# batra-mlp-lab/visdial

Hardware: NVIDIA H100
Metric: QA-rounds/sec mn-att-ques-im-hist+disc train step (higher is better)
Workload: dtype f16 operands + f16 saved state for the option LSTM, tf32 operands elsewhere; fp32 accumulate, fp32 cell state / gradients / optimiser

## Files before the change

visdial_b200/csrc/lstm16.cu:

```cuda
#include <cuda.h>
#include <cuda_fp16.h>
#include <map>
#include <mutex>
#include "../../include/visdial_b200.h"
#include "kernels.cuh"
#include "tc_ptx.cuh"

namespace vd {
namespace tc {

constexpr int BM16 = 128;
constexpr int BK16 = 64;
constexpr int UK16 = 16;
constexpr int BN16 = 128;
constexpr int EW16 = 8;
constexpr int STAGE16 = 32768;

__device__ __forceinline__ float tanh16(float x) { float y; asm("tanh.approx.f32 %0, %1;" : "=f"(y) : "f"(x)); return y; }
__device__ __forceinline__ float sig16(float x) { return fmaf(0.5f, tanh16(0.5f * x), 0.5f); }

__device__ __forceinline__ uint32_t pack2(float a, float b) {
  uint32_t r;
  asm("{\n .reg .f16 lo, hi;\n cvt.rn.satfinite.f16.f32 lo, %1;\n cvt.rn.satfinite.f16.f32 hi, %2;\n mov.b32 %0, {lo, hi};\n}"
      : "=r"(r) : "f"(a), "f"(b));
// ... 20 lines not shown
  unsigned lo = __shfl_sync(0xffffffffu, (unsigned)v, src_lane), hi = __shfl_sync(0xffffffffu, (unsigned)(v >> 32), src_lane);
  return (const void*)(((unsigned long long)hi << 32) | lo);
}
__device__ __forceinline__ void cp16(void* dst, const void* src) {
  asm volatile("cp.async.cg.shared.global [%0], [%1], 16;" ::"r"(smem_u32(dst)), "l"(src) : "memory");
}
__device__ __forceinline__ void t16_load(uint8_t* base, const void* mine, int lane) {
#pragma unroll
  for (int ps = 0; ps < 2; ++ps) {
    const int row = ps * 8 + (lane >> 2), c = lane & 3;
    const uint8_t* src = (const uint8_t*)shfl_vptr(mine, row);
    uint8_t* dst = base + row * 64 + ((c ^ ((row >> 1) & 3)) << 4);
    if (src) cp16(dst, src + c * 16); else *reinterpret_cast<uint4*>(dst) = make_uint4(0, 0, 0, 0);
  }
}
__device__ __forceinline__ void t32_load(uint8_t* base, const void* mine, int lane) {
#pragma unroll
  for (int ps = 0; ps < 4; ++ps) {
    const int row = ps * 4 + (lane >> 3), c = lane & 7;
    const uint8_t* src = (const uint8_t*)shfl_vptr(mine, row);
    uint8_t* dst = base + row * 128 + ((c ^ (row & 7)) << 4);
    if (src) cp16(dst, src + c * 16); else *reinterpret_cast<float4*>(dst) = make_float4(0.f, 0.f, 0.f, 0.f);
  }
}
__device__ __forceinline__ void cp_wait_all() {
  asm volatile("cp.async.wait_all;" ::: "memory");
  __syncwarp();
}
__device__ __forceinline__ float2 ld_h2(uint8_t* p) { return __half22float2(*reinterpret_cast<const __half2*>(p)); }
__device__ __forceinline__ void st_h2(uint8_t* p, float a, float b) { *reinterpret_cast<uint32_t*>(p) = pack2(a, b); }

struct Lstm16Params {
  int R, H;
  const __half* ptable; const int32_t* tok;
  const float* bias;
  const float* c_prev;
  const int32_t* mask_ids;
  float* h32_out;
  int save_gates;
  const __half* gsave; const float* c_cur; float* dc_carry;
};
struct Lstm16Maps { CUtensorMap g16, c, h16; };

template <int MODE>
struct Cfg16 {
  static constexpr int THREADS = 128 + 32 * EW16;
  static constexpr int STG_PER_WARP = MODE == 0 ? (5 * T16_BYTES + T32_BYTES) : (4 * T16_BYTES + 3 * T32_BYTES);
  static constexpr int STG_BYTES = EW16 * STG_PER_WARP;
  static constexpr int STAGES = (232448 - 1024 - 256 - STG_BYTES) / STAGE16;
  static constexpr int TOTAL = STAGES * STAGE16 + STG_BYTES + 1024 + 256;
};

template <int MODE>
__global__ void __launch_bounds__(Cfg16<MODE>::THREADS, 1)
k_lstm16(const __grid_constant__ CUtensorMap tmA, const __grid_constant__ CUtensorMap tmB,
         const __grid_constant__ Lstm16Maps em, const Lstm16Params p) {
  using C = Cfg16<MODE>;
  constexpr int STAGES = C::STAGES;
  extern __shared__ uint8_t smem_raw[];
  uint8_t* smem = (uint8_t*)(((uintptr_t)smem_raw + 1023) & ~(uintptr_t)1023);
  uint8_t* stg_all = smem + STAGES * STAGE16;
  uint64_t* full = (uint64_t*)(stg_all + C::STG_BYTES);
  uint64_t* empty = full + STAGES;

  const int warp = threadIdx.x >> 5, lane = threadIdx.x & 31;
  const int H = p.H;
  const int num_m = (p.R + BM16 - 1) / BM16;
  const int num_n = MODE == 0 ? H / 32 : H / BN16;
  const int num_tiles = num_m * num_n;
  const int num_kb = (MODE == 0 ? H : 4 * H) / BK16;

  if (threadIdx.x == 0) {
    for (int s = 0; s < STAGES; ++s) { mbar_init(&full[s], 1); mbar_init(&empty[s], 2); }
    asm volatile("fence.mbarrier_init.release.cluster;" ::: "memory");
  }
  __syncthreads();

  if (warp < 4) {
    if (threadIdx.x == 0) {
      int s = 0; uint32_t ph = 0;
      for (int tile = blockIdx.x; tile < num_tiles; tile += gridDim.x) {
        const int m0 = (tile / num_n) * BM16;
        const int nt = tile % num_n;
        for (int kb = 0; kb < num_kb; ++kb) {
          mbar_wait(&empty[s], ph ^ 1);
          uint8_t* sa = smem + s * STAGE16;
          uint8_t* sb = sa + 16384;
          mbar_expect_tx(&full[s], STAGE16);
          tma_load_2d(sa, &tmA, &full[s], kb * BK16, m0);
          if (MODE == 0) {
#pragma unroll
            for (int g = 0; g < 4; ++g) tma_load_2d(sb + g * 4096, &tmB, &full[s], kb * BK16, g * H + nt * 32);
          } else {
            tma_load_2d(sb, &tmB, &full[s], kb * BK16, nt * BN16);
          }
          if (++s == STAGES) { s = 0; ph ^= 1; }
        }
      }
    }
  } else {
    const int cw = warp - 4, wg = cw >> 2;
    uint8_t* stg = stg_all + cw * C::STG_PER_WARP;
    const int fr = lane >> 2, fu = 2 * (lane & 3);
    int s = 0; uint32_t ph = 0;
    auto contract = [&](float (&d)[BN16 / 2]) {
#pragma unroll
      for (int i = 0; i < BN16 / 2; ++i) d[i] = 0.f;
      int prev = -1;
      for (int kb = 0; kb < num_kb; ++kb) {
        mbar_wait(&full[s], ph);
        const uint32_t sa = smem_u32(smem + s * STAGE16);
        const uint64_t adesc = make_desc(sa + wg * 64 * 128, 16, 1024), bdesc = make_desc(sa + 16384, 16, 1024);
        wgmma_fence();
#pragma unroll
        for (int k = 0; k < BK16 / UK16; ++k)
          wgmma_f16_n128(d, adesc + (uint64_t)(k * 2), bdesc + (uint64_t)(k * 2), (kb | k) ? 1u : 0u);
        wgmma_commit();
        wgmma_wait<1>();
        if (prev >= 0 && (threadIdx.x & 127) == 0) mbar_arrive(&empty[prev]);
        prev = s;
        if (++s == STAGES) { s = 0; ph ^= 1; }
      }
      wgmma_wait<0>();
      wgmma_hold(d);
      if (prev >= 0 && (threadIdx.x & 127) == 0) mbar_arrive(&empty[prev]);
    };
    if constexpr (MODE == 0) {
      uint8_t* sG = stg; uint8_t* sH = stg + 4 * T16_BYTES; uint8_t* sC = sH + T16_BYTES;
      for (int tile = blockIdx.x; tile < num_tiles; tile += gridDim.x) {
        const int m0 = (tile / num_n) * BM16;
        const int nt = tile % num_n;
        const int r0 = m0 + wg * 64 + (cw & 3) * 16;
        const int j0 = nt * 32;
        const int64_t row = (int64_t)r0 + (lane & 15);
        const bool row_ok = row < p.R;
        const float keep = (row_ok && p.mask_ids && p.mask_ids[row] == 0) ? 0.f : 1.f;
        const int32_t tk = row_ok ? __ldg(p.tok + row) : 0;
        const __half* prow = tk != 0 ? p.ptable + (int64_t)tk * 4 * H + j0 : nullptr;
        const float* cprow = (row_ok && p.c_prev) ? p.c_prev + row * H + j0 : nullptr;
        if (lane == 0) bulk_wait_read0();
        __syncwarp();
#pragma unroll
        for (int g = 0; g < 4; ++g) t16_load(sG + g * T16_BYTES, prow ? prow + g * H : nullptr, lane);
        t32_load(sC, cprow, lane);
        float d[BN16 / 2];
        contract(d);
        cp_wait_all();
#pragma unroll
        for (int hh = 0; hh < 2; ++hh) {
          const int r = fr + 8 * hh;
          const float kp = __shfl_sync(0xffffffffu, keep, r);
          const int64_t grow = (int64_t)r0 + r;
#pragma unroll
          for (int jj = 0; jj < 4; ++jj) {
            const int u = 8 * jj + fu;
            float a[4][2], cp[2], hn[2];
#pragma unroll
            for (int g = 0; g < 4; ++g) {
              const float2 x = ld_h2(t16_at(sG + g * T16_BYTES, r, u));
              const float2 b = __ldg(reinterpret_cast<const float2*>(p.bias + g * H + j0 + u));
              a[g][0] = d[4 * (jj + 4 * g) + 2 * hh] + (x.x + b.x);
              a[g][1] = d[4 * (jj + 4 * g) + 2 * hh + 1] + (x.y + b.y);
            }
            const float2 c2 = *reinterpret_cast<const float2*>(t32_at(sC, r, u));
            cp[0] = c2.x; cp[1] = c2.y;
#pragma unroll
            for (int e = 0; e < 2; ++e) {
              const float gi = sig16(a[0][e]), gf = sig16(a[1][e]), go = sig16(a[2][e]), gg = tanh16(a[3][e]);
              const float c_ = (gf * cp[e] + gi * gg) * kp;
              a[0][e] = gi * kp; a[1][e] = gf * kp; a[2][e] = go * kp; a[3][e] = gg * kp;
              cp[e] = c_; hn[e] = go * tanh16(c_) * kp;
            }
#pragma unroll
            for (int g = 0; g < 4; ++g) st_h2(t16_at(sG + g * T16_BYTES, r, u), a[g][0], a[g][1]);
            *reinterpret_cast<float2*>(t32_at(sC, r, u)) = make_float2(cp[0], cp[1]);
            st_h2(t16_at(sH, r, u), hn[0], hn[1]);
            if (p.h32_out && grow < p.R)
              *reinterpret_cast<float2*>(p.h32_out + grow * H + j0 + u) = make_float2(hn[0], hn[1]);
          }
        }
        fence_proxy_async_smem();
        __syncwarp();
        if (lane == 0) {
          if (p.save_gates) {
#pragma unroll
            for (int g = 0; g < 4; ++g) tma_store_2d(&em.g16, sG + g * T16_BYTES, g * H + j0, r0);
          }
          tma_store_2d(&em.c, sC, j0, r0);
          tma_store_2d(&em.h16, sH, j0, r0);
          bulk_commit();
        }
        __syncwarp();
      }
    } else {
      uint8_t* sG = stg; uint8_t* sCP = stg + 4 * T16_BYTES; uint8_t* sCC = sCP + T32_BYTES; uint8_t* sDC = sCC + T32_BYTES;
      for (int tile = blockIdx.x; tile < num_tiles; tile += gridDim.x) {
        const int m0 = (tile / num_n) * BM16;
        const int nt = tile % num_n;
        const int r0 = m0 + wg * 64 + (cw & 3) * 16;
        const int64_t row = (int64_t)r0 + (lane & 15);
        const bool row_ok = row < p.R;
        const float keep = (row_ok && p.mask_ids && p.mask_ids[row] == 0) ? 0.f : 1.f;
        const __half* grow = row_ok ? p.gsave + row * 4 * H : nullptr;
        const float* cprow = (row_ok && p.c_prev) ? p.c_prev + row * H : nullptr;
        const float* ccrow = row_ok ? p.c_cur + row * H : nullptr;
        const float* dcrow = row_ok ? p.dc_carry + row * H : nullptr;
        auto fetch = [&](int j) {
          if (lane == 0) bulk_wait_read0();
          __syncwarp();
#pragma unroll
          for (int g = 0; g < 4; ++g) t16_load(sG + g * T16_BYTES, grow ? grow + g * H + j : nullptr, lane);
          t32_load(sCP, cprow ? cprow + j : nullptr, lane);
          t32_load(sCC, ccrow ? ccrow + j : nullptr, lane);
          t32_load(sDC, dcrow ? dcrow + j : nullptr, lane);
        };
        fetch(nt * BN16);
        float d[BN16 / 2];
        contract(d);
#pragma unroll
        for (int grp = 0; grp < BN16 / 32; ++grp) {
          const int j = nt * BN16 + grp * 32;
          if (grp > 0) fetch(j);
          cp_wait_all();
#pragma unroll
          for (int hh = 0; hh < 2; ++hh) {
            const int r = fr + 8 * hh;
            const float keep_r = __shfl_sync(0xffffffffu, keep, r);
#pragma unroll
            for (int jj = 0; jj < 4; ++jj) {
              const int u = 8 * jj + fu;
              float g[4][2], cp[2], cc[2], dc[2], out[4][2], dcn[2];
#pragma unroll
              for (int gg = 0; gg < 4; ++gg) {
                const float2 x = ld_h2(t16_at(sG + gg * T16_BYTES, r, u));
                g[gg][0] = x.x; g[gg][1] = x.y;
              }
              const float2 cp2 = *reinterpret_cast<const float2*>(t32_at(sCP, r, u));
              const float2 cc2 = *reinterpret_cast<const float2*>(t32_at(sCC, r, u));
              const float2 dc2 = *reinterpret_cast<const float2*>(t32_at(sDC, r, u));
              cp[0] = cp2.x; cp[1] = cp2.y; cc[0] = cc2.x; cc[1] = cc2.y; dc[0] = dc2.x; dc[1] = dc2.y;
#pragma unroll
              for (int e = 0; e < 2; ++e) {
                const float dh = d[4 * (4 * grp + jj) + 2 * hh + e];
                const float gi = g[0][e], gf = g[1][e], go = g[2][e], gg_ = g[3][e];
                const float tcv = tanh16(cc[e]);
                const float dd = (dc[e] + dh * go * (1.f - tcv * tcv)) * keep_r;
                const float dhe = dh * keep_r;
                out[0][e] = dd * gg_ * gi * (1.f - gi);
                out[1][e] = dd * cp[e] * gf * (1.f - gf);
                out[2][e] = dhe * tcv * go * (1.f - go);
                out[3][e] = dd * gi * (1.f - gg_ * gg_);
                dcn[e] = dd * gf;
              }
#pragma unroll
              for (int gg = 0; gg < 4; ++gg) st_h2(t16_at(sG + gg * T16_BYTES, r, u), out[gg][0], out[gg][1]);
              *reinterpret_cast<float2*>(t32_at(sDC, r, u)) = make_float2(dcn[0], dcn[1]);
            }
          }
          fence_proxy_async_smem();
          __syncwarp();
          if (lane == 0) {
#pragma unroll
            for (int gg = 0; gg < 4; ++gg) tma_store_2d(&em.g16, sG + gg * T16_BYTES, gg * H + j, r0);
            tma_store_2d(&em.c, sDC, j, r0);
            bulk_commit();
          }
          __syncwarp();
        }
      }
    }
    if (lane == 0) asm volatile("cp.async.bulk.wait_group 0;" ::: "memory");
  }
}

constexpr int A16_KB = 64;
constexpr int A16_BM = 128, A16_BN = 256;
constexpr int A16_THREADS = 384;
constexpr int A16_A_BYTES = (A16_BM / 64) * A16_KB * 128;
constexpr int A16_B_BYTES = (A16_BN / 64) * A16_KB * 128;
constexpr int A16_STAGE = A16_A_BYTES + A16_B_BYTES;
constexpr int A16_STAGES = 4;
constexpr int A16_TOTAL = A16_STAGES * A16_STAGE + 1024 + 256;
constexpr int A16_CHUNKS_PER_CTA = 24;
constexpr int A16_MIN_CHUNK = 32;
struct Atb16Params {
  int M, N, tiles_n, tiles, kbt;
  int chunk, num_chunks;
  float* C; int64_t ldc; const float* inv_scale;
  int* counter;
};

// ... 258 lines not shown
#pragma unroll
      for (int e = 0; e < 8; ++e) acc[e] += v[e];
    }
    flush(cur);
  }
}

static CUtensorMap make_tmap16(const void* base, CUtensorMapDataType dt, int esize, int64_t rows, int64_t cols, int64_t ld,
                               int box_rows, int box_cols, CUtensorMapSwizzle swz) {
  CUtensorMap tm;
  cuuint64_t dims[2] = {(cuuint64_t)cols, (cuuint64_t)rows};
  cuuint64_t strides[1] = {(cuuint64_t)ld * esize};
  cuuint32_t box[2] = {(cuuint32_t)box_cols, (cuuint32_t)box_rows};
  cuuint32_t estr[2] = {1, 1};
  CUresult r = get_encode()(&tm, dt, 2, (void*)base, dims, strides, box, estr, CU_TENSOR_MAP_INTERLEAVE_NONE, swz,
                            CU_TENSOR_MAP_L2_PROMOTION_L2_256B, CU_TENSOR_MAP_FLOAT_OOB_FILL_NONE);
  if (r != CUDA_SUCCESS) {
    char buf[256];
    snprintf(buf, sizeof(buf), "cuTensorMapEncodeTiled (lstm16) failed (%d): base %p rows %lld cols %lld ld %lld box %dx%d", (int)r, base,
             (long long)rows, (long long)cols, (long long)ld, box_rows, box_cols);
    throw CudaError(-3, buf);
  }
  return tm;
}
static CUtensorMap tmap_h(const __half* base, int64_t rows, int64_t cols, int64_t ld, int box_rows, int box_cols,
                          CUtensorMapSwizzle swz) {
  return make_tmap16(base, CU_TENSOR_MAP_DATA_TYPE_FLOAT16, 2, rows, cols, ld, box_rows, box_cols, swz);
}
static CUtensorMap tmap_f(const float* base, int64_t rows, int64_t cols, int64_t ld, int box_rows, int box_cols,
                          CUtensorMapSwizzle swz) {
  return make_tmap16(base, CU_TENSOR_MAP_DATA_TYPE_FLOAT32, 4, rows, cols, ld, box_rows, box_cols, swz);
}

template <int MODE>
static void launch16(LaunchCtx& cx, const CUtensorMap& tA, const CUtensorMap& tB, const Lstm16Maps& em, const Lstm16Params& p,
                     int num_tiles) {
  using C = Cfg16<MODE>;
  static bool attr_set = false;
  if (!attr_set) {
    VD_CUDA_CHECK(cudaFuncSetAttribute(k_lstm16<MODE>, cudaFuncAttributeMaxDynamicSharedMemorySize, C::TOTAL));
    attr_set = true;
  }
  const int pmax = cx.sms();
  int grid = num_tiles;
  if (num_tiles > pmax) { const int rounds = cdiv(num_tiles, pmax); grid = cdiv(num_tiles, rounds); }
  k_lstm16<MODE><<<grid, C::THREADS, C::TOTAL, cx.stream>>>(tA, tB, em, p);
  check_launch(cx, "k_lstm16");
}

}

bool lstm16_shape_ok(int64_t R, int H) { return H % 256 == 0 && H <= 512 && R >= 1024; }

void lstm16_step_fwd(LaunchCtx& cx, int64_t R, int H, const __half* h_prev16, const __half* Wh16, const __half* ptable16,
                     const int32_t* tok, const float* bias, const float* c_prev, const int32_t* mask_ids, __half* gates16,
                     float* c_out, __half* h16_out, float* h32_out) {
  using namespace tc;
  VD_REQUIRE(lstm16_shape_ok(R, H), VD_E_STATE, "lstm16_step_fwd: shape");
  Lstm16Params p = {};
  p.R = (int)R; p.H = H; p.ptable = ptable16; p.tok = tok; p.bias = bias; p.c_prev = c_prev; p.mask_ids = mask_ids;
  p.h32_out = h32_out; p.save_gates = gates16 != nullptr;
  CUtensorMap tA = tmap_h(h_prev16, R, H, H, BM16, BK16, CU_TENSOR_MAP_SWIZZLE_128B);
  CUtensorMap tB = tmap_h(Wh16, 4 * (int64_t)H, H, H, 32, BK16, CU_TENSOR_MAP_SWIZZLE_128B);
  Lstm16Maps em;
  em.g16 = gates16 ? tmap_h(gates16, R, 4 * (int64_t)H, 4 * (int64_t)H, 16, 32, CU_TENSOR_MAP_SWIZZLE_64B)
                   : tmap_h(h16_out, R, H, H, 16, 32, CU_TENSOR_MAP_SWIZZLE_64B);
  em.c = tmap_f(c_out, R, H, H, 16, 32, CU_TENSOR_MAP_SWIZZLE_128B);
  em.h16 = tmap_h(h16_out, R, H, H, 16, 32, CU_TENSOR_MAP_SWIZZLE_64B);
  launch16<0>(cx, tA, tB, em, p, cdiv(R, BM16) * (H / 32));
}

void lstm16_step_bwd(LaunchCtx& cx, int64_t R, int H, const __half* da_next16, const __half* Whb16, const __half* gates16,
                     const float* c_prev, const float* c_cur, float* dc_carry, const int32_t* mask_ids, __half* da16) {
  using namespace tc;
  VD_REQUIRE(lstm16_shape_ok(R, H), VD_E_STATE, "lstm16_step_bwd: shape");
  Lstm16Params p = {};
  p.R = (int)R; p.H = H; p.gsave = gates16; p.c_prev = c_prev; p.c_cur = c_cur; p.dc_carry = dc_carry; p.mask_ids = mask_ids;
  CUtensorMap tA = tmap_h(da_next16, R, 4 * (int64_t)H, 4 * (int64_t)H, BM16, BK16, CU_TENSOR_MAP_SWIZZLE_128B);
// ... 18 lines not shown
  const int64_t n = R * (H / 8);
  tc::k_lstm16_bwd_last<<<(unsigned)((n + 255) / 256), 256, 0, cx.stream>>>(gates16, c_prev, c_cur, dh_last, scale, mask_ids,
                                                                             dc_carry, da16, R, H);
  check_launch(cx, "k_lstm16_bwd_last");
}

void cvt_f32_to_f16(LaunchCtx& cx, __half* dst, int64_t ldd, const float* src, int64_t lds, int64_t rows, int cols) {
  VD_REQUIRE(cols % 4 == 0 && lds % 4 == 0 && ldd % 4 == 0, VD_E_STATE, "cvt_f32_to_f16: alignment");
  const int64_t n = rows * (cols / 4);
  if (n == 0) return;
  tc::k_cvt16<<<(unsigned)((n + 255) / 256), 256, 0, cx.stream>>>(dst, ldd, src, lds, rows, cols);
  check_launch(cx, "k_cvt16");
}

void pick_grad_scale(LaunchCtx& cx, const float* x, int64_t n, uint32_t* bits, float* scale2) {
  VD_REQUIRE(n % 4 == 0, VD_E_STATE, "pick_grad_scale: n % 4");
  VD_CUDA_CHECK(cudaMemsetAsync(bits, 0, sizeof(uint32_t), cx.stream));
  const int blocks = (int)std::min<int64_t>((n / 4 + 255) / 256, 4 * cx.sm_count);
  tc::k_amax<<<blocks, 256, 0, cx.stream>>>(x, n / 4, bits);
  check_launch(cx, "k_amax");
  tc::k_pick_scale<<<1, 1, 0, cx.stream>>>(bits, scale2);
  check_launch(cx, "k_pick_scale");
}

void segsum_rows16(LaunchCtx& cx, const __half* X, int64_t ldx, const int32_t* perm, const int32_t* sorted_tok, int64_t n,
                   float* out, int ncols, const float* inv_scale) {
  VD_REQUIRE(ncols % 8 == 0 && ldx % 8 == 0, VD_E_STATE, "segsum_rows16: alignment");
  if (n == 0) return;
  tc::k_segsum16<<<(unsigned)((n + tc::SEG16_ROWS - 1) / tc::SEG16_ROWS), 256, 0, cx.stream>>>(X, ldx, perm, sorted_tok, n, out, ncols,
                                                                                               inv_scale);
  check_launch(cx, "k_segsum16");
}

static int* atb16_counter(cudaStream_t stream) {
  static std::mutex mu;
  static std::map<std::pair<int, cudaStream_t>, int*> counters;
  int dev = 0;
  VD_CUDA_CHECK(cudaGetDevice(&dev));
  std::lock_guard<std::mutex> lock(mu);
  int*& c = counters[{dev, stream}];
  if (!c) {
    VD_CUDA_CHECK(cudaMalloc((void**)&c, 2 * sizeof(int)));
    VD_CUDA_CHECK(cudaMemsetAsync(c, 0, 2 * sizeof(int), stream));
  }
  return c;
}

void gemm_atb16(LaunchCtx& cx, int M, int N, int64_t K, const __half* A, int64_t lda, const __half* B, int64_t ldb, float* C,
                int64_t ldc, const float* inv_scale) {
  using namespace tc;
  VD_REQUIRE(M % 64 == 0 && N % 64 == 0 && K >= A16_KB && lda % 8 == 0 && ldb % 8 == 0, VD_E_STATE, "gemm_atb16: shape");
  Atb16Params p = {};
  p.M = M; p.N = N; p.tiles_n = cdiv(N, A16_BN); p.tiles = cdiv(M, A16_BM) * p.tiles_n;
  VD_REQUIRE((K + A16_KB - 1) / A16_KB <= INT32_MAX, VD_E_STATE, "gemm_atb16: K");
  p.kbt = (int)((K + A16_KB - 1) / A16_KB);
  const int64_t sms = cx.sms(), total = (int64_t)p.tiles * p.kbt;
  p.chunk = (int)std::min<int64_t>(p.kbt, std::max<int64_t>(A16_MIN_CHUNK, cdiv(total, sms * A16_CHUNKS_PER_CTA)));
  p.num_chunks = p.tiles * cdiv(p.kbt, p.chunk);
  p.C = C; p.ldc = ldc; p.inv_scale = inv_scale;
  p.counter = atb16_counter(cx.stream);
  CUtensorMap tA = tmap_h(A, K, M, lda, A16_KB, 64, CU_TENSOR_MAP_SWIZZLE_128B),
              tB = tmap_h(B, K, N, ldb, A16_KB, 64, CU_TENSOR_MAP_SWIZZLE_128B);
  static bool attr_set = false;
  if (!attr_set) {
    VD_CUDA_CHECK(cudaFuncSetAttribute(k_atb16<true>, cudaFuncAttributeMaxDynamicSharedMemorySize, A16_TOTAL));
    VD_CUDA_CHECK(cudaFuncSetAttribute(k_atb16<false>, cudaFuncAttributeMaxDynamicSharedMemorySize, A16_TOTAL));
    attr_set = true;
  }
  const unsigned grid = (unsigned)std::min<int64_t>(sms, p.num_chunks);
  if (ldc % 4 == 0 && ((uintptr_t)C & 15) == 0) k_atb16<true><<<grid, A16_THREADS, A16_TOTAL, cx.stream>>>(tA, tB, p);
  else k_atb16<false><<<grid, A16_THREADS, A16_TOTAL, cx.stream>>>(tA, tB, p);
  check_launch(cx, "k_atb16");
}

}
```

visdial_b200/csrc/tc_ptx.cuh:

```cuda
#pragma once
#include <cuda.h>
#include <stdint.h>

namespace vd {
namespace tc {

__device__ __forceinline__ uint32_t smem_u32(const void* p) { return (uint32_t)__cvta_generic_to_shared(p); }

__device__ __forceinline__ void mbar_init(uint64_t* bar, uint32_t count) {
  asm volatile("mbarrier.init.shared::cta.b64 [%0], %1;" ::"r"(smem_u32(bar)), "r"(count));
}
__device__ __forceinline__ void mbar_expect_tx(uint64_t* bar, uint32_t bytes) {
  asm volatile("mbarrier.arrive.expect_tx.shared::cta.b64 _, [%0], %1;" ::"r"(smem_u32(bar)), "r"(bytes) : "memory");
}
__device__ __forceinline__ void mbar_arrive(uint64_t* bar) {
  asm volatile("mbarrier.arrive.shared::cta.b64 _, [%0];" ::"r"(smem_u32(bar)) : "memory");
}
__device__ __forceinline__ void mbar_wait(uint64_t* bar, uint32_t parity) {
  uint32_t done = 0, spins = 0;
  uint32_t addr = smem_u32(bar);
  while (!done) {
    asm volatile(
        "{\n .reg .pred p;\n mbarrier.try_wait.parity.shared::cta.b64 p, [%1], %2;\n selp.u32 %0, 1, 0, p;\n}"
        : "=r"(done) : "r"(addr), "r"(parity) : "memory");
    if (!done && ++spins > (1u << 24)) __trap();
  }
}
__device__ __forceinline__ void tma_load_2d(void* smem_dst, const CUtensorMap* tm, uint64_t* bar, int c0, int c1) {
  asm volatile(
      "cp.async.bulk.tensor.2d.shared::cluster.global.mbarrier::complete_tx::bytes [%0], [%1, {%3, %4}], [%2];"
      ::"r"(smem_u32(smem_dst)), "l"(tm), "r"(smem_u32(bar)), "r"(c0), "r"(c1) : "memory");
}
__device__ __forceinline__ void wgmma_fence() { asm volatile("wgmma.fence.sync.aligned;" ::: "memory"); }
__device__ __forceinline__ void wgmma_commit() { asm volatile("wgmma.commit_group.sync.aligned;" ::: "memory"); }
template <int N> __device__ __forceinline__ void wgmma_wait() { asm volatile("wgmma.wait_group.sync.aligned %0;" ::"n"(N) : "memory"); }
template <int NR> __device__ __forceinline__ void wgmma_hold(float (&d)[NR]) {
#pragma unroll
  for (int i = 0; i < NR; ++i) asm volatile("" : "+f"(d[i])::"memory");
}
__device__ __forceinline__ void bar_named(int id, int threads) { asm volatile("bar.sync %0, %1;" ::"r"(id), "r"(threads) : "memory"); }

__device__ __forceinline__ uint64_t make_desc(uint32_t saddr, uint32_t lbo_bytes, uint32_t sbo_bytes) {
  uint64_t d = 0;
  d |= (uint64_t)((saddr & 0x3FFFF) >> 4);
  d |= (uint64_t)((lbo_bytes >> 4) & 0x3FFF) << 16;
  d |= (uint64_t)((sbo_bytes >> 4) & 0x3FFF) << 32;
  d |= (uint64_t)1 << 62;
  return d;
}

__device__ __forceinline__ void wgmma_tf32_n32(float (&d)[16], uint64_t a, uint64_t b, uint32_t acc) {
  asm volatile(
      "{\n .reg .pred p;\n setp.ne.b32 p, %18, 0;\n"
      "wgmma.mma_async.sync.aligned.m64n32k8.f32.tf32.tf32 {%0, %1, %2, %3, %4, %5, %6, %7, %8, %9, %10, %11, %12, %13, %14, %15}, %16, %17, p, 1, 1;\n}\n"
      : "+f"(d[0]), "+f"(d[1]), "+f"(d[2]), "+f"(d[3]), "+f"(d[4]), "+f"(d[5]), "+f"(d[6]), "+f"(d[7]), "+f"(d[8]), "+f"(d[9]), "+f"(d[10]), "+f"(d[11]), "+f"(d[12]), "+f"(d[13]), "+f"(d[14]), "+f"(d[15])
      : "l"(a), "l"(b), "r"(acc));
}

__device__ __forceinline__ void wgmma_tf32_n64(float (&d)[32], uint64_t a, uint64_t b, uint32_t acc) {
  asm volatile(
      "{\n .reg .pred p;\n setp.ne.b32 p, %34, 0;\n"
      "wgmma.mma_async.sync.aligned.m64n64k8.f32.tf32.tf32 {%0, %1, %2, %3, %4, %5, %6, %7, %8, %9, %10, %11, %12, %13, %14, %15, %16, %17, %18, %19, %20, %21, %22, %23, %24, %25, %26, %27, %28, %29, %30, %31}, %32, %33, p, 1, 1;\n}\n"
      : "+f"(d[0]), "+f"(d[1]), "+f"(d[2]), "+f"(d[3]), "+f"(d[4]), "+f"(d[5]), "+f"(d[6]), "+f"(d[7]), "+f"(d[8]), "+f"(d[9]), "+f"(d[10]), "+f"(d[11]), "+f"(d[12]), "+f"(d[13]), "+f"(d[14]), "+f"(d[15]), "+f"(d[16]), "+f"(d[17]), "+f"(d[18]), "+f"(d[19]), "+f"(d[20]), "+f"(d[21]), "+f"(d[22]), "+f"(d[23]), "+f"(d[24]), "+f"(d[25]), "+f"(d[26]), "+f"(d[27]), "+f"(d[28]), "+f"(d[29]), "+f"(d[30]), "+f"(d[31])
      : "l"(a), "l"(b), "r"(acc));
}

__device__ __forceinline__ void wgmma_tf32_n128(float (&d)[64], uint64_t a, uint64_t b, uint32_t acc) {
  asm volatile(
      "{\n .reg .pred p;\n setp.ne.b32 p, %66, 0;\n"
      "wgmma.mma_async.sync.aligned.m64n128k8.f32.tf32.tf32 {%0, %1, %2, %3, %4, %5, %6, %7, %8, %9, %10, %11, %12, %13, %14, %15, %16, %17, %18, %19, %20, %21, %22, %23, %24, %25, %26, %27, %28, %29, %30, %31, %32, %33, %34, %35, %36, %37, %38, %39, %40, %41, %42, %43, %44, %45, %46, %47, %48, %49, %50, %51, %52, %53, %54, %55, %56, %57, %58, %59, %60, %61, %62, %63}, %64, %65, p, 1, 1;\n}\n"
      : "+f"(d[0]), "+f"(d[1]), "+f"(d[2]), "+f"(d[3]), "+f"(d[4]), "+f"(d[5]), "+f"(d[6]), "+f"(d[7]), "+f"(d[8]), "+f"(d[9]), "+f"(d[10]), "+f"(d[11]), "+f"(d[12]), "+f"(d[13]), "+f"(d[14]), "+f"(d[15]), "+f"(d[16]), "+f"(d[17]), "+f"(d[18]), "+f"(d[19]), "+f"(d[20]), "+f"(d[21]), "+f"(d[22]), "+f"(d[23]), "+f"(d[24]), "+f"(d[25]), "+f"(d[26]), "+f"(d[27]), "+f"(d[28]), "+f"(d[29]), "+f"(d[30]), "+f"(d[31]), "+f"(d[32]), "+f"(d[33]), "+f"(d[34]), "+f"(d[35]), "+f"(d[36]), "+f"(d[37]), "+f"(d[38]), "+f"(d[39]), "+f"(d[40]), "+f"(d[41]), "+f"(d[42]), "+f"(d[43]), "+f"(d[44]), "+f"(d[45]), "+f"(d[46]), "+f"(d[47]), "+f"(d[48]), "+f"(d[49]), "+f"(d[50]), "+f"(d[51]), "+f"(d[52]), "+f"(d[53]), "+f"(d[54]), "+f"(d[55]), "+f"(d[56]), "+f"(d[57]), "+f"(d[58]), "+f"(d[59]), "+f"(d[60]), "+f"(d[61]), "+f"(d[62]), "+f"(d[63])
      : "l"(a), "l"(b), "r"(acc));
// ... 72 lines not shown
```

visdial_b200/csrc/engine.h:

```cpp
#pragma once
#include <functional>
#include <string>
#include <vector>
#include "../../include/visdial_b200.h"
#include "kernels.cuh"

namespace vd {

enum EncKind { ENC_LF_QUES = 0, ENC_LF_QIH = 1, ENC_HREA = 2, ENC_MN_ATT = 3, ENC_LF_QI = 4, ENC_LF_QH = 5, ENC_HRE_QH = 6, ENC_HRE_QIH = 7,
               ENC_MN_QH = 8, ENC_MN_QIH = 9, ENC_LF_ATT = 10 };
enum DecKind { DEC_DISC = 0, DEC_GEN = 1 };

struct Cfg {
  std::string encoder, decoder;
  int enc = 0, dec = 0;
  int V = 0, E = 300, H = 512, L = 2, F = 4096, S = 14, IE = 300, Cm = 512, hops = 1, R = 10, K = 100;
  float dropout = 0.5f;
  int gpuid = 0;
  bool useIm = false, useHist = false, att = false;
  bool fam_lf = false, fam_hre = false, fam_mn = false;
  bool hre_att = false;
  bool san = false;
  bool img_in_q = false;
  bool img_drop = false;
// ... 153 lines not shown
  DropCfg dropcfg(float p) const;
  void gemm_tn(int M, int N, int K, const float* A, int64_t lda, const int32_t* gather, const float* B, int64_t ldb,
               float* C, int64_t ldc, float beta, const float* bias, int act);
  void gemm_atb(int M, int N, int64_t K, const float* A, int64_t lda, const int32_t* gather, const float* B, int64_t ldb,
                float* C, int64_t ldc);
  void linear_fwd(int wseg, const float* x, int64_t rows, float* y, int act);
  void linear_bwd(int wseg, const float* x, const float* dy, int64_t rows, float* dx, float beta_dx);
  void refresh_shadows();
  void stage_batch(const vd_batch* b);
  LstmRoute route_lstm(int64_t R, int H, bool gathered, bool has_h0, const float* WhT, int64_t ldw, const float* Wh) const;
  LstmRoute route_lstm(const LstmRun& r) const {
    return route_lstm(r.R, r.H, r.gather != nullptr, r.h0 != nullptr, Wtp(r.wseg) + r.D, r.D + r.H,
                      Wp(r.wseg) + (int64_t)r.D * 4 * r.H);
  }
  void route_lstm_pair(LstmRun& l1, LstmRun& l2) const;
  void lstm_simt_fwd_step(const LstmFwdStep& s);
  int lstm_tc_fwd_step(const LstmFwdStep& s);
  void lstm_simt_bwd_step(const LstmBwdStep& s);
  int lstm_tc_bwd_step(const LstmBwdStep& s);
  void lstm_forward(LstmRun& r, bool save);
  void lstm_forward_begin(LstmRun& r, bool save, bool xproj_by_caller = false);
  void lstm_forward_step(LstmRun& r, int t, bool xproj_by_caller = false);
  void lstm_xproj(const LstmRun& r, int t0, int nt, float* gates);
  void lstm_backward_begin(LstmRun& r, const float* dh_all, const float* dh_last, const float* dc_last);
  void lstm_backward_step(LstmRun& r, int t);
  void lstm_backward_end(LstmRun& r, float* dx_out, float* dh0_out, float* dc0_out);
  void lstm_pair_forward(LstmRun& l1, LstmRun& l2, const PairStreams& s);
  void lstm_pair_backward(LstmRun& l1, LstmRun& l2, const float* dh_last2, const float* dc_last2, const float* dh_last1,
                          const float* dc_last1, float* dx1_out, const PairStreams& s);
  bool serial_pairs() const { return cfg.useHist && hist1.route.fwd == LstmPath::Pair16; }
  cudaStream_t opt_stream = nullptr;
  cudaEvent_t ev_opt_fork = nullptr, ev_opt_done = nullptr;
  bool opt_overlap = true, opt_fwd_pending = false, opt_bwd_pending = false;
  int opt_reserve_sms = 16;
  float* opt_demb = nullptr;
  void options_forward_async();
  void options_backward(const float* dfeat);
  void join_options_backward();
  const int32_t* dense_round = nullptr;
  GrowBuf dense_buf[2];
  float forward_backward_dense(const vd_batch* b, const int32_t* round_host, const float* relevance_host);
  std::vector<cudaEvent_t> ev_pool;
  cudaEvent_t pool_event(size_t i);
  void lstm_backward(LstmRun& r, const float* dh_all, const float* dh_last, const float* dc_last, float* dx_out,
                     float* dh0_out, float* dc0_out);

  void encoder_forward(const vd_batch* b);
  void encoder_backward(const float* dEnc);
  float *qi_join = nullptr, *qi_proj = nullptr;
  const float* mn_query_in = nullptr;
  void mn_block_fwd(const float* qin, const float* h3, float* out);
  void mn_block_bwd(const float* dout, const float* out, float* dqin, float* dh3);
  void san_block_fwd(const float* u0);
  void san_block_bwd(const float* dEnc, float* du0);
  void forward_connect();
  void decoder_forward();
  float criterion_forward();
  void criterion_backward();
  void decoder_backward();
  const float* backward_connect();
  void retrieve(const vd_batch* b, int use_gt, int32_t* ranks_host);
  void gen_option_lhood();
  LstmRun gstep1, gstep2;
  float* gstep_logp = nullptr;
  void gen_decoder_step(int64_t rows, const int32_t* tokens_host, const float* const* h_prev, const float* const* c_prev);
  void gen_decoder_step_logits(int64_t rows, const int32_t* tok, const float* const* h_prev, const float* const* c_prev);
  void gen_beam_search(int k, int L, int start_token, int end_token, int32_t* answer_host, int32_t* length_host, double* score_host);
// ... 43 lines not shown
```

Baseline: 16150.

## Split option-LSTM kernel into dedicated MMA and epilogue warpgroups with smem accumulator handoff

Adds a separate MMA warpgroup that computes both 64-row halves of the 128x128 tile and hands the fp32 accumulators to eight epilogue warps through a shared-memory buffer guarded by full/empty mbarriers. The aim is to overlap the gate nonlinearity and backward epilogue of one tile with the tensor-core contraction of the next. Registers are rebalanced with setmaxnreg, and in backward mode c_prev is read directly into registers instead of being staged. The accumulator buffer takes shared memory, which can reduce the number of pipeline stages, and the single accumulator buffer still serialises MMA against epilogue reads.

```diff
diff --git a/visdial_b200/csrc/lstm16.cu b/visdial_b200/csrc/lstm16.cu
--- a/visdial_b200/csrc/lstm16.cu
+++ b/visdial_b200/csrc/lstm16.cu
@@ -88,12 +88,44 @@
 
 template <int MODE>
 struct Cfg16 {
-  static constexpr int THREADS = 128 + 32 * EW16;
-  static constexpr int STG_PER_WARP = MODE == 0 ? (5 * T16_BYTES + T32_BYTES) : (4 * T16_BYTES + 3 * T32_BYTES);
+  static constexpr int THREADS = 256 + 32 * EW16;
+  static constexpr int STG_PER_WARP = MODE == 0 ? (5 * T16_BYTES + T32_BYTES) : (4 * T16_BYTES + 2 * T32_BYTES);
   static constexpr int STG_BYTES = EW16 * STG_PER_WARP;
-  static constexpr int STAGES = (232448 - 1024 - 256 - STG_BYTES) / STAGE16;
-  static constexpr int TOTAL = STAGES * STAGE16 + STG_BYTES + 1024 + 256;
+  static constexpr int ACC_BYTES = BM16 * BN16 * 4;
+  static constexpr int STAGES = (232448 - 1024 - 256 - STG_BYTES - ACC_BYTES) / STAGE16;
+  static constexpr int TOTAL = STAGES * STAGE16 + ACC_BYTES + STG_BYTES + 1024 + 256;
 };
+
+template <int STAGES>
+__device__ __forceinline__ void contract16(float (&d)[2][BN16 / 2], uint8_t* smem, uint64_t* full, uint64_t* empty, int& s,
+                                           uint32_t& ph, int num_kb) {
+#pragma unroll
+  for (int j = 0; j < 2; ++j)
+#pragma unroll
+    for (int i = 0; i < BN16 / 2; ++i) d[j][i] = 0.f;
+  int prev = -1;
+  for (int kb = 0; kb < num_kb; ++kb) {
+    mbar_wait(&full[s], ph);
+    const uint32_t sa = smem_u32(smem + s * STAGE16);
+    const uint64_t bdesc = make_desc(sa + 16384, 16, 1024);
+    wgmma_fence();
+#pragma unroll
+    for (int k = 0; k < BK16 / UK16; ++k)
+#pragma unroll
+      for (int j = 0; j < 2; ++j)
+        wgmma_f16_n128(d[j], make_desc(sa + j * 64 * 128, 16, 1024) + (uint64_t)(k * 2), bdesc + (uint64_t)(k * 2),
+                       (kb | k) ? 1u : 0u);
+    wgmma_commit();
+    wgmma_wait<1>();
+    if (prev >= 0 && (threadIdx.x & 127) == 0) mbar_arrive(&empty[prev]);
+    prev = s;
+    if (++s == STAGES) { s = 0; ph ^= 1; }
+  }
+  wgmma_wait<0>();
+#pragma unroll
+  for (int j = 0; j < 2; ++j) wgmma_hold(d[j]);
+  if (prev >= 0 && (threadIdx.x & 127) == 0) mbar_arrive(&empty[prev]);
+}
 
 template <int MODE>
 __global__ void __launch_bounds__(Cfg16<MODE>::THREADS, 1)
@@ -103,9 +135,12 @@
   constexpr int STAGES = C::STAGES;
   extern __shared__ uint8_t smem_raw[];
   uint8_t* smem = (uint8_t*)(((uintptr_t)smem_raw + 1023) & ~(uintptr_t)1023);
-  uint8_t* stg_all = smem + STAGES * STAGE16;
+  float2* accbuf = (float2*)(smem + STAGES * STAGE16);
+  uint8_t* stg_all = smem + STAGES * STAGE16 + C::ACC_BYTES;
   uint64_t* full = (uint64_t*)(stg_all + C::STG_BYTES);
   uint64_t* empty = full + STAGES;
+  uint64_t* acc_full = empty + STAGES;
+  uint64_t* acc_empty = acc_full + 1;
 
   const int warp = threadIdx.x >> 5, lane = threadIdx.x & 31;
   const int H = p.H;
@@ -115,12 +150,15 @@
   const int num_kb = (MODE == 0 ? H : 4 * H) / BK16;
 
   if (threadIdx.x == 0) {
-    for (int s = 0; s < STAGES; ++s) { mbar_init(&full[s], 1); mbar_init(&empty[s], 2); }
+    for (int s = 0; s < STAGES; ++s) { mbar_init(&full[s], 1); mbar_init(&empty[s], 1); }
+    mbar_init(acc_full, 128);
+    mbar_init(acc_empty, 32 * EW16);
     asm volatile("fence.mbarrier_init.release.cluster;" ::: "memory");
   }
   __syncthreads();
 
   if (warp < 4) {
+    setmaxnreg_dec<40>();
     if (threadIdx.x == 0) {
       int s = 0; uint32_t ph = 0;
       for (int tile = blockIdx.x; tile < num_tiles; tile += gridDim.x) {
@@ -142,33 +180,28 @@
         }
       }
     }
+  } else if (warp < 8) {
+    setmaxnreg_inc<168>();
+    float2* mine = accbuf + ((warp - 4) * (BN16 / 4)) * 32 + lane;
+    int s = 0; uint32_t ph = 0, aph = 0;
+    for (int tile = blockIdx.x; tile < num_tiles; tile += gridDim.x) {
+      float d[2][BN16 / 2];
+      contract16<STAGES>(d, smem, full, empty, s, ph, num_kb);
+      mbar_wait(acc_empty, aph ^ 1);
+#pragma unroll
+      for (int e = 0; e < 2; ++e)
+#pragma unroll
+        for (int q = 0; q < BN16 / 4; ++q) mine[(e * 4 * (BN16 / 4) + q) * 32] = make_float2(d[e][2 * q], d[e][2 * q + 1]);
+      mbar_arrive(acc_full);
+      aph ^= 1;
+    }
   } else {
-    const int cw = warp - 4, wg = cw >> 2;
+    setmaxnreg_inc<152>();
+    const int cw = warp - 8, wg = cw >> 2;
     uint8_t* stg = stg_all + cw * C::STG_PER_WARP;
     const int fr = lane >> 2, fu = 2 * (lane & 3);
-    int s = 0; uint32_t ph = 0;
-    auto contract = [&](float (&d)[BN16 / 2]) {
-#pragma unroll
-      for (int i = 0; i < BN16 / 2; ++i) d[i] = 0.f;
-      int prev = -1;
-      for (int kb = 0; kb < num_kb; ++kb) {
-        mbar_wait(&full[s], ph);
-        const uint32_t sa = smem_u32(smem + s * STAGE16);
-        const uint64_t adesc = make_desc(sa + wg * 64 * 128, 16, 1024), bdesc = make_desc(sa + 16384, 16, 1024);
-        wgmma_fence();
-#pragma unroll
-        for (int k = 0; k < BK16 / UK16; ++k)
-          wgmma_f16_n128(d, adesc + (uint64_t)(k * 2), bdesc + (uint64_t)(k * 2), (kb | k) ? 1u : 0u);
-        wgmma_commit();
-        wgmma_wait<1>();
-        if (prev >= 0 && (threadIdx.x & 127) == 0) mbar_arrive(&empty[prev]);
-        prev = s;
-        if (++s == STAGES) { s = 0; ph ^= 1; }
-      }
-      wgmma_wait<0>();
-      wgmma_hold(d);
-      if (prev >= 0 && (threadIdx.x & 127) == 0) mbar_arrive(&empty[prev]);
-    };
+    const float2* theirs = accbuf + (cw * (BN16 / 4)) * 32 + lane;
+    uint32_t aph = 0;
     if constexpr (MODE == 0) {
       uint8_t* sG = stg; uint8_t* sH = stg + 4 * T16_BYTES; uint8_t* sC = sH + T16_BYTES;
       for (int tile = blockIdx.x; tile < num_tiles; tile += gridDim.x) {
@@ -187,8 +220,8 @@
 #pragma unroll
         for (int g = 0; g < 4; ++g) t16_load(sG + g * T16_BYTES, prow ? prow + g * H : nullptr, lane);
         t32_load(sC, cprow, lane);
-        float d[BN16 / 2];
-        contract(d);
+        mbar_wait(acc_full, aph);
+        aph ^= 1;
         cp_wait_all();
 #pragma unroll
         for (int hh = 0; hh < 2; ++hh) {
@@ -203,8 +236,9 @@
             for (int g = 0; g < 4; ++g) {
               const float2 x = ld_h2(t16_at(sG + g * T16_BYTES, r, u));
               const float2 b = __ldg(reinterpret_cast<const float2*>(p.bias + g * H + j0 + u));
-              a[g][0] = d[4 * (jj + 4 * g) + 2 * hh] + (x.x + b.x);
-              a[g][1] = d[4 * (jj + 4 * g) + 2 * hh + 1] + (x.y + b.y);
+              const float2 d = theirs[(2 * (jj + 4 * g) + hh) * 32];
+              a[g][0] = d.x + (x.x + b.x);
+              a[g][1] = d.y + (x.y + b.y);
             }
             const float2 c2 = *reinterpret_cast<const float2*>(t32_at(sC, r, u));
             cp[0] = c2.x; cp[1] = c2.y;
@@ -223,6 +257,7 @@
               *reinterpret_cast<float2*>(p.h32_out + grow * H + j0 + u) = make_float2(hn[0], hn[1]);
           }
         }
+        mbar_arrive(acc_empty);
         fence_proxy_async_smem();
         __syncwarp();
         if (lane == 0) {
@@ -237,7 +272,7 @@
         __syncwarp();
       }
     } else {
-      uint8_t* sG = stg; uint8_t* sCP = stg + 4 * T16_BYTES; uint8_t* sCC = sCP + T32_BYTES; uint8_t* sDC = sCC + T32_BYTES;
+      uint8_t* sG = stg; uint8_t* sCC = stg + 4 * T16_BYTES; uint8_t* sDC = sCC + T32_BYTES;
       for (int tile = blockIdx.x; tile < num_tiles; tile += gridDim.x) {
         const int m0 = (tile / num_n) * BM16;
         const int nt = tile % num_n;
@@ -246,21 +281,28 @@
         const bool row_ok = row < p.R;
         const float keep = (row_ok && p.mask_ids && p.mask_ids[row] == 0) ? 0.f : 1.f;
         const __half* grow = row_ok ? p.gsave + row * 4 * H : nullptr;
-        const float* cprow = (row_ok && p.c_prev) ? p.c_prev + row * H : nullptr;
         const float* ccrow = row_ok ? p.c_cur + row * H : nullptr;
         const float* dcrow = row_ok ? p.dc_carry + row * H : nullptr;
+        float2 cpr[2][4];
         auto fetch = [&](int j) {
           if (lane == 0) bulk_wait_read0();
           __syncwarp();
 #pragma unroll
           for (int g = 0; g < 4; ++g) t16_load(sG + g * T16_BYTES, grow ? grow + g * H + j : nullptr, lane);
-          t32_load(sCP, cprow ? cprow + j : nullptr, lane);
           t32_load(sCC, ccrow ? ccrow + j : nullptr, lane);
           t32_load(sDC, dcrow ? dcrow + j : nullptr, lane);
+#pragma unroll
+          for (int hh = 0; hh < 2; ++hh) {
+            const int64_t fr_row = (int64_t)r0 + fr + 8 * hh;
+#pragma unroll
+            for (int jj = 0; jj < 4; ++jj)
+              cpr[hh][jj] = (p.c_prev && fr_row < p.R) ? *reinterpret_cast<const float2*>(p.c_prev + fr_row * H + j + 8 * jj + fu)
+                                                       : make_float2(0.f, 0.f);
+          }
         };
         fetch(nt * BN16);
-        float d[BN16 / 2];
-        contract(d);
+        mbar_wait(acc_full, aph);
+        aph ^= 1;
 #pragma unroll
         for (int grp = 0; grp < BN16 / 32; ++grp) {
           const int j = nt * BN16 + grp * 32;
@@ -279,13 +321,14 @@
                 const float2 x = ld_h2(t16_at(sG + gg * T16_BYTES, r, u));
                 g[gg][0] = x.x; g[gg][1] = x.y;
               }
-              const float2 cp2 = *reinterpret_cast<const float2*>(t32_at(sCP, r, u));
+              const float2 cp2 = cpr[hh][jj];
               const float2 cc2 = *reinterpret_cast<const float2*>(t32_at(sCC, r, u));
               const float2 dc2 = *reinterpret_cast<const float2*>(t32_at(sDC, r, u));
               cp[0] = cp2.x; cp[1] = cp2.y; cc[0] = cc2.x; cc[1] = cc2.y; dc[0] = dc2.x; dc[1] = dc2.y;
+              const float2 d2 = theirs[(2 * (4 * grp + jj) + hh) * 32];
 #pragma unroll
               for (int e = 0; e < 2; ++e) {
-                const float dh = d[4 * (4 * grp + jj) + 2 * hh + e];
+                const float dh = e ? d2.y : d2.x;
                 const float gi = g[0][e], gf = g[1][e], go = g[2][e], gg_ = g[3][e];
                 const float tcv = tanh16(cc[e]);
                 const float dd = (dc[e] + dh * go * (1.f - tcv * tcv)) * keep_r;
@@ -301,6 +344,7 @@
               *reinterpret_cast<float2*>(t32_at(sDC, r, u)) = make_float2(dcn[0], dcn[1]);
             }
           }
+          if (grp == BN16 / 32 - 1) mbar_arrive(acc_empty);
           fence_proxy_async_smem();
           __syncwarp();
           if (lane == 0) {
diff --git a/visdial_b200/csrc/tc_ptx.cuh b/visdial_b200/csrc/tc_ptx.cuh
--- a/visdial_b200/csrc/tc_ptx.cuh
+++ b/visdial_b200/csrc/tc_ptx.cuh
@@ -38,6 +38,8 @@
 #pragma unroll
   for (int i = 0; i < NR; ++i) asm volatile("" : "+f"(d[i])::"memory");
 }
+template <int N> __device__ __forceinline__ void setmaxnreg_dec() { asm volatile("setmaxnreg.dec.sync.aligned.u32 %0;" ::"n"(N)); }
+template <int N> __device__ __forceinline__ void setmaxnreg_inc() { asm volatile("setmaxnreg.inc.sync.aligned.u32 %0;" ::"n"(N)); }
 __device__ __forceinline__ void bar_named(int id, int threads) { asm volatile("bar.sync %0, %1;" ::"r"(id), "r"(threads) : "memory"); }
 
 __device__ __forceinline__ uint64_t make_desc(uint32_t saddr, uint32_t lbo_bytes, uint32_t sbo_bytes) {
```

Measured after the change: 16870, median of 6. +4.5%, better.

## Use atomic work-claiming tile scheduler in fp16 LSTM kernel and shrink option SM reserve

Applied to the files above, without the earlier changes.

The fp16 LSTM step kernel no longer assigns tiles statically by block index. The producer thread claims tiles from a global atomic counter and passes each tile id to the consumer warps through a per-stage shared-memory tag, ending with a -1 sentinel; the last block to finish resets the counter. This lets CTAs that start late, for example because the options stream is occupying SMs, pick up less work, so the tail is more balanced. The number of SMs reserved for the overlapped option stream also drops from 16 to 4. The cost is atomics on every tile claim and a counter now shared with the atb16 GEMM on the same stream.

```diff
diff --git a/visdial_b200/csrc/engine.h b/visdial_b200/csrc/engine.h
--- a/visdial_b200/csrc/engine.h
+++ b/visdial_b200/csrc/engine.h
@@ -209,7 +209,7 @@
   cudaStream_t opt_stream = nullptr;
   cudaEvent_t ev_opt_fork = nullptr, ev_opt_done = nullptr;
   bool opt_overlap = true, opt_fwd_pending = false, opt_bwd_pending = false;
-  int opt_reserve_sms = 16;
+  int opt_reserve_sms = 4;
   float* opt_demb = nullptr;
   void options_forward_async();
   void options_backward(const float* dfeat);
diff --git a/visdial_b200/csrc/lstm16.cu b/visdial_b200/csrc/lstm16.cu
--- a/visdial_b200/csrc/lstm16.cu
+++ b/visdial_b200/csrc/lstm16.cu
@@ -76,6 +76,7 @@
 
 struct Lstm16Params {
   int R, H;
+  int* counter;
   const __half* ptable; const int32_t* tok;
   const float* bias;
   const float* c_prev;
@@ -106,6 +107,7 @@
   uint8_t* stg_all = smem + STAGES * STAGE16;
   uint64_t* full = (uint64_t*)(stg_all + C::STG_BYTES);
   uint64_t* empty = full + STAGES;
+  int* tag = (int*)(empty + STAGES);
 
   const int warp = threadIdx.x >> 5, lane = threadIdx.x & 31;
   const int H = p.H;
@@ -123,13 +125,16 @@
   if (warp < 4) {
     if (threadIdx.x == 0) {
       int s = 0; uint32_t ph = 0;
-      for (int tile = blockIdx.x; tile < num_tiles; tile += gridDim.x) {
+      for (;;) {
+        const int tile = atomicAdd(p.counter, 1);
+        if (tile >= num_tiles) break;
         const int m0 = (tile / num_n) * BM16;
         const int nt = tile % num_n;
         for (int kb = 0; kb < num_kb; ++kb) {
           mbar_wait(&empty[s], ph ^ 1);
           uint8_t* sa = smem + s * STAGE16;
           uint8_t* sb = sa + 16384;
+          if (kb == 0) tag[s] = tile;
           mbar_expect_tx(&full[s], STAGE16);
           tma_load_2d(sa, &tmA, &full[s], kb * BK16, m0);
           if (MODE == 0) {
@@ -140,6 +145,14 @@
           }
           if (++s == STAGES) { s = 0; ph ^= 1; }
         }
+      }
+      mbar_wait(&empty[s], ph ^ 1);
+      tag[s] = -1;
+      mbar_arrive(&full[s]);
+      __threadfence();
+      if (atomicAdd(p.counter + 1, 1) == (int)gridDim.x - 1) {
+        atomicExch(p.counter, 0);
+        atomicExch(p.counter + 1, 0);
       }
     }
   } else {
@@ -169,9 +182,10 @@
       wgmma_hold(d);
       if (prev >= 0 && (threadIdx.x & 127) == 0) mbar_arrive(&empty[prev]);
     };
+    auto next_tile = [&]() { mbar_wait(&full[s], ph); return tag[s]; };
     if constexpr (MODE == 0) {
       uint8_t* sG = stg; uint8_t* sH = stg + 4 * T16_BYTES; uint8_t* sC = sH + T16_BYTES;
-      for (int tile = blockIdx.x; tile < num_tiles; tile += gridDim.x) {
+      for (int tile = next_tile(); tile >= 0; tile = next_tile()) {
         const int m0 = (tile / num_n) * BM16;
         const int nt = tile % num_n;
         const int r0 = m0 + wg * 64 + (cw & 3) * 16;
@@ -238,7 +252,7 @@
       }
     } else {
       uint8_t* sG = stg; uint8_t* sCP = stg + 4 * T16_BYTES; uint8_t* sCC = sCP + T32_BYTES; uint8_t* sDC = sCC + T32_BYTES;
-      for (int tile = blockIdx.x; tile < num_tiles; tile += gridDim.x) {
+      for (int tile = next_tile(); tile >= 0; tile = next_tile()) {
         const int m0 = (tile / num_n) * BM16;
         const int nt = tile % num_n;
         const int r0 = m0 + wg * 64 + (cw & 3) * 16;
@@ -625,8 +639,22 @@
   return make_tmap16(base, CU_TENSOR_MAP_DATA_TYPE_FLOAT32, 4, rows, cols, ld, box_rows, box_cols, swz);
 }
 
+static int* claim_counter(cudaStream_t stream) {
+  static std::mutex mu;
+  static std::map<std::pair<int, cudaStream_t>, int*> counters;
+  int dev = 0;
+  VD_CUDA_CHECK(cudaGetDevice(&dev));
+  std::lock_guard<std::mutex> lock(mu);
+  int*& c = counters[{dev, stream}];
+  if (!c) {
+    VD_CUDA_CHECK(cudaMalloc((void**)&c, 2 * sizeof(int)));
+    VD_CUDA_CHECK(cudaMemsetAsync(c, 0, 2 * sizeof(int), stream));
+  }
+  return c;
+}
+
 template <int MODE>
-static void launch16(LaunchCtx& cx, const CUtensorMap& tA, const CUtensorMap& tB, const Lstm16Maps& em, const Lstm16Params& p,
+static void launch16(LaunchCtx& cx, const CUtensorMap& tA, const CUtensorMap& tB, const Lstm16Maps& em, Lstm16Params p,
                      int num_tiles) {
   using C = Cfg16<MODE>;
   static bool attr_set = false;
@@ -634,9 +662,8 @@
     VD_CUDA_CHECK(cudaFuncSetAttribute(k_lstm16<MODE>, cudaFuncAttributeMaxDynamicSharedMemorySize, C::TOTAL));
     attr_set = true;
   }
-  const int pmax = cx.sms();
-  int grid = num_tiles;
-  if (num_tiles > pmax) { const int rounds = cdiv(num_tiles, pmax); grid = cdiv(num_tiles, rounds); }
+  p.counter = claim_counter(cx.stream);
+  const int grid = cdiv(num_tiles, cdiv(num_tiles, cx.sms()));
   k_lstm16<MODE><<<grid, C::THREADS, C::TOTAL, cx.stream>>>(tA, tB, em, p);
   check_launch(cx, "k_lstm16");
 }
@@ -721,20 +748,6 @@
   check_launch(cx, "k_segsum16");
 }
 
-static int* atb16_counter(cudaStream_t stream) {
-  static std::mutex mu;
-  static std::map<std::pair<int, cudaStream_t>, int*> counters;
-  int dev = 0;
-  VD_CUDA_CHECK(cudaGetDevice(&dev));
-  std::lock_guard<std::mutex> lock(mu);
-  int*& c = counters[{dev, stream}];
-  if (!c) {
-    VD_CUDA_CHECK(cudaMalloc((void**)&c, 2 * sizeof(int)));
-    VD_CUDA_CHECK(cudaMemsetAsync(c, 0, 2 * sizeof(int), stream));
-  }
-  return c;
-}
-
 void gemm_atb16(LaunchCtx& cx, int M, int N, int64_t K, const __half* A, int64_t lda, const __half* B, int64_t ldb, float* C,
                 int64_t ldc, const float* inv_scale) {
   using namespace tc;
@@ -747,7 +760,7 @@
   p.chunk = (int)std::min<int64_t>(p.kbt, std::max<int64_t>(A16_MIN_CHUNK, cdiv(total, sms * A16_CHUNKS_PER_CTA)));
   p.num_chunks = p.tiles * cdiv(p.kbt, p.chunk);
   p.C = C; p.ldc = ldc; p.inv_scale = inv_scale;
-  p.counter = atb16_counter(cx.stream);
+  p.counter = claim_counter(cx.stream);
   CUtensorMap tA = tmap_h(A, K, M, lda, A16_KB, 64, CU_TENSOR_MAP_SWIZZLE_128B),
               tB = tmap_h(B, K, N, ldb, A16_KB, 64, CU_TENSOR_MAP_SWIZZLE_128B);
   static bool attr_set = false;
```

Result: faster. 16130 before, 16590 after (median of 6 runs) (+2.9%).
